# henrycharlesworth/settlers_of_catan_RL

Hardware: AMD Instinct MI355X
Metric: Catan env-steps/sec at 65k parallel games (higher is better)
Workload: dtype u8/u32 (integer bitboards)

## Files before the change

settlers_of_catan_rl_amd/csrc/catan_abi.hip:

```cpp
#include <hip/hip_runtime.h>

#include <cstdio>
#include <cstring>
#include <new>
#include <string>
#include <vector>

#include "../../include/catan_hip.h"
#include "../../include/catan_hip_nn.h"
#include "../../include/catan_hip_tuning.h"
#include "catan_kernels.hip"
#include "catan_obs.hip"
#include "catan_ppo.hip"
#include "catan_nn.hip"
#include "catan_tile_encoder.hip"
#include "catan_heads.hip"
#include "catan_collector.hip"
#include "catan_rows.hip"
#include "catan_te_bwd.hip"
#include "catan_optim.hip"
#include "catan_wgrad_big.hip"

using namespace catan;

struct catan_env {
    int device;
    long n, N;
    Ctx ctx;
    catan_cfg_t cfg;
    void* state;
    u32* mpk;
    u32* spec_state;
    u32* spec_mpk;
    u32 spec_epoch;
    int ctr_clean;
    int lock_parity;
    u32* err;
    double* reward64;
    i32* scratch_actions;
    float* scratch_reward;
    u8* scratch_done;
    Pending pend;
    unsigned long long* prof;
    int prof_on;
    int lr_mid_budget;
    int lr_mid_heavy_grid;
    int t1_group;
    int g_open, g_slot, g_passes; int64_t g_count;
    int lr_split;
    int step_bin_order;
    int step_wpb;
    u32* prof_wave;
    u32* pctr;
    int lr_budget[3];
    int lr_round[2];
    int deferred_fused;
    int fused_subs;
    int step_games;
    hipStream_t side;
    hipEvent_t ev_fork, ev_join;
    hipStream_t fstream[2];
    hipEvent_t ev_fready[3], ev_fdone[3];
    float* f_reward;
    u8* f_done;
    hipStream_t sstream;
    hipEvent_t ev_sdone[2];
    float* s_reward;
    u8* s_done;
    int64_t d_it;
    int d_window;
    hipStream_t d_stream;
    MtPair* mt_dev;
};

constexpr int DEFAULT_STEP_WAVE_GAMES = 32;
constexpr int DEFAULT_FUSED_SUBS = 8;
constexpr int LR_BUDGET_DEFERRED = 12;
constexpr int T1_STAGGER_US = 4, LR_GRID_FUSED = 4096, LR_BUDGET_FUSED = 10;
constexpr unsigned EV_SYNC = hipEventDisableTiming | hipEventDisableSystemFence;
static thread_local std::string g_err;
static int fail(int code, const std::string& msg) { g_err = msg; return code; }
#define HIPCHK(x)                                                                                    \
    do {                                                                                             \
        hipError_t e_ = (x);                                                                         \
        if (e_ != hipSuccess) return fail(CATAN_EHIP, std::string(#x) + ": " + hipGetErrorString(e_)); \
    } while (0)

template <class T>
static int attn_dispatch(bool bwd, const void* qkv, const int* lens, const void* dout, void* out, long B, int L, int H, int HD, hipStream_t st) {
    const T* q = (const T*)qkv;
    const bool mfma = sizeof(T) == 2 && (((uintptr_t)qkv | (uintptr_t)out | (uintptr_t)dout) & 15) == 0;
    const unsigned nb4 = (unsigned)((B + 3) / 4);
    const unsigned short* q16 = (const unsigned short*)qkv;
    if (L == 19 && H == 4 && HD == 16) {
        unsigned nb = (unsigned)((B + 2) / 3);
        if (mfma && !bwd) hipLaunchKernelGGL((k_attn_mfma_fwd<19, 4, 16>), dim3(nb4), dim3(256), 0, st, q16, lens, (unsigned short*)out, B);
        else if (mfma && lens) hipLaunchKernelGGL((k_attn_mfma_bwd<19, 4, 16, true>), dim3(nb4), dim3(256), 0, st, q16, lens, (const unsigned short*)dout, (unsigned short*)out, B);
        else if (mfma) hipLaunchKernelGGL((k_attn_mfma_bwd<19, 4, 16, false>), dim3(nb4), dim3(256), 0, st, q16, lens, (const unsigned short*)dout, (unsigned short*)out, B);
        else if (!bwd) hipLaunchKernelGGL((k_attn_fwd<T, 19, 4, 16>), dim3(nb), dim3(64), 0, st, q, lens, (T*)out, B);
        else hipLaunchKernelGGL((k_attn_bwd<T, 19, 4, 16>), dim3(nb), dim3(64), 0, st, q, lens, (const T*)dout, (T*)out, B);
    } else if (L == 25 && H == 4 && HD == 4) {
        unsigned nb = (unsigned)((B + 1) / 2);
        if (mfma && !bwd) hipLaunchKernelGGL((k_attn_mfma_fwd<25, 4, 4>), dim3(nb4), dim3(256), 0, st, q16, lens, (unsigned short*)out, B);
        else if (mfma && lens) hipLaunchKernelGGL((k_attn_mfma_bwd<25, 4, 4, true>), dim3(nb4), dim3(256), 0, st, q16, lens, (const unsigned short*)dout, (unsigned short*)out, B);
        else if (mfma) hipLaunchKernelGGL((k_attn_mfma_bwd<25, 4, 4, false>), dim3(nb4), dim3(256), 0, st, q16, lens, (const unsigned short*)dout, (unsigned short*)out, B);
        else if (!bwd) hipLaunchKernelGGL((k_attn_fwd<T, 25, 4, 4>), dim3(nb), dim3(64), 0, st, q, lens, (T*)out, B);
        else hipLaunchKernelGGL((k_attn_bwd<T, 25, 4, 4>), dim3(nb), dim3(64), 0, st, q, lens, (const T*)dout, (T*)out, B);
    } else return fail(CATAN_EINVAL, "catan_attention: unsupported (L, heads, head_dim); built for (19,4,16) and (25,4,4)");
    HIPCHK(hipGetLastError());
    return CATAN_OK;
}
template <class T, int D, int GL>
static int ln_launch(bool bwd, const void* x, const float* w, const float* b, const void* dy, void* out, float* dw, float* db,
                     long rows, float eps, int relu, hipStream_t st) {
    long nb = (rows + (256 / GL) - 1) / (256 / GL);
    const long cap = bwd ? 2048 : 8192;
    if (nb > cap) nb = cap;
    if (!bwd) hipLaunchKernelGGL((k_ln_fwd<T, D, GL>), dim3((unsigned)nb), dim3(256), 0, st, (const T*)x, w, b, (T*)out, rows, eps, relu);
    else hipLaunchKernelGGL((k_ln_bwd<T, D, GL>), dim3((unsigned)nb), dim3(256), 0, st, (const T*)x, w, b, (const T*)dy, (T*)out, dw, db, rows, eps, relu);
    HIPCHK(hipGetLastError());
    return CATAN_OK;
}
template <class T, int EPL, int GL>
static int lnw_launch(bool bwd, const void* x, const float* w, const float* b, const void* dy, void* out, float* dw, float* db,
                      long rows, float eps, int relu, hipStream_t st) {
    constexpr int RPB = 256 / GL;
    long nb = (rows + RPB - 1) / RPB;
    const long cap = bwd ? 1024 : 8192;
    if (nb > cap) nb = cap;
// ... 196 lines not shown
    if (cfg) e->cfg = *cfg; else catan_cfg_default(&e->cfg);
    size_t bytes = (size_t)e->N * STATE_BYTES_PER_GAME;
    hipError_t rc = hipMalloc(&e->state, bytes);
    if (rc == hipSuccess) rc = hipMalloc((void**)&e->mpk, (size_t)e->N * MPK_STRIDE * sizeof(u32));
    if (rc == hipSuccess) rc = hipMalloc((void**)&e->spec_state, (size_t)e->N * REC * sizeof(u32));
    if (rc == hipSuccess) rc = hipMalloc((void**)&e->spec_mpk, (size_t)e->N * MPK_STRIDE * sizeof(u32));
    if (rc == hipSuccess) rc = hipMalloc((void**)&e->err, 64);
    if (rc == hipSuccess) rc = hipMalloc((void**)&e->scratch_actions, (size_t)e->n * ACTION_WORDS * sizeof(i32));
    if (rc == hipSuccess) rc = hipMalloc((void**)&e->scratch_reward, (size_t)e->n * 4 * sizeof(float));
    if (rc == hipSuccess) rc = hipMalloc((void**)&e->scratch_done, (size_t)e->n);
    if (rc == hipSuccess) rc = hipMalloc((void**)&e->pend.ctr, CTR_WORDS * sizeof(u32));
    if (rc == hipSuccess) rc = hipMalloc((void**)&e->pend.req[0], (size_t)e->N * sizeof(u64));
    if (rc == hipSuccess) rc = hipMalloc((void**)&e->pend.req[1], (size_t)e->N * sizeof(u64));
    if (rc == hipSuccess) rc = hipMalloc((void**)&e->pend.req[2], (size_t)e->N * sizeof(u64));
    if (rc == hipSuccess) rc = hipMalloc((void**)&e->f_reward, (size_t)e->n * 4 * sizeof(float));
    if (rc == hipSuccess) rc = hipMalloc((void**)&e->f_done, (size_t)e->n);
    int lr_cus = getenv("CATAN_LR_CUS") ? atoi(getenv("CATAN_LR_CUS")) : 0;
    if (rc == hipSuccess && lr_cus > 0) {
        hipDeviceProp_t prop; int dev = 0;
        int cus = (hipGetDevice(&dev) == hipSuccess && hipGetDeviceProperties(&prop, dev) == hipSuccess) ? prop.multiProcessorCount : 256;
        if (lr_cus > cus) lr_cus = cus;
        std::vector<uint32_t> mask((cus + 31) / 32, 0u);
        const char* pat = getenv("CATAN_LR_CUS_PATTERN");
        for (int k = 0; k < lr_cus; k++) { const int b = (pat && pat[0] == 'b') ? k : (int)((long)k * cus / lr_cus); mask[b >> 5] |= 1u << (b & 31); }
        rc = hipExtStreamCreateWithCUMask(&e->fstream[0], (uint32_t)mask.size(), mask.data());
    } else if (rc == hipSuccess) rc = hipStreamCreateWithFlags(&e->fstream[0], hipStreamNonBlocking);
    e->fstream[1] = e->fstream[0];
    for (int i = 0; i < 3 && rc == hipSuccess; i++) {
        rc = hipEventCreateWithFlags(&e->ev_fready[i], EV_SYNC);
        if (rc == hipSuccess) rc = hipEventCreateWithFlags(&e->ev_fdone[i], EV_SYNC);
    }
    for (int i = 0; i < 2 && rc == hipSuccess; i++) {
        rc = hipMalloc((void**)&e->pend.heavy[i], (size_t)e->N * sizeof(u64));
        if (rc == hipSuccess) rc = hipMalloc((void**)&e->pend.resets[i][0], (size_t)e->N * sizeof(i32));
        if (rc == hipSuccess) rc = hipMalloc((void**)&e->pend.resets[i][1], (size_t)e->N * sizeof(i32));
        if (rc == hipSuccess) rc = hipMalloc((void**)&e->pend.resets[i][2], (size_t)e->N * sizeof(i32));
        if (rc == hipSuccess) rc = hipEventCreateWithFlags(&e->ev_sdone[i], EV_SYNC);
    }
    if (rc == hipSuccess) rc = hipMalloc((void**)&e->pend.heavy2, (size_t)e->N * sizeof(u64));
    if (rc == hipSuccess) rc = hipStreamCreateWithFlags(&e->sstream, hipStreamNonBlocking);
    if (rc == hipSuccess) rc = hipMalloc((void**)&e->s_reward, (size_t)e->n * 4 * sizeof(float));
    if (rc == hipSuccess) rc = hipMalloc((void**)&e->s_done, (size_t)e->n);
    e->fused_subs = DEFAULT_FUSED_SUBS;
    if (const char* fs = getenv("CATAN_FUSED_SUBS")) { const int v = atoi(fs); if (v == 1 || v == 2 || v == 4 || v == 8 || v == 16) e->fused_subs = v; }
    static_assert(DEFAULT_FUSED_SUBS <= MAX_SUBS, "sub-lists per bin");
    if (rc == hipSuccess) rc = hipMalloc((void**)&e->pend.lists, (size_t)BIN_SETS * NBINS * e->fused_subs * e->N * sizeof(i32));
    if (rc == hipSuccess) rc = hipMalloc((void**)&e->pend.bctr, (size_t)BIN_SETS * NBINS * MAX_SUBS * BCTR_PAD * sizeof(u32));
    if (rc == hipSuccess) rc = hipStreamCreateWithFlags(&e->side, hipStreamNonBlocking);
    if (rc == hipSuccess) rc = hipEventCreateWithFlags(&e->ev_fork, EV_SYNC);
    if (rc == hipSuccess) rc = hipEventCreateWithFlags(&e->ev_join, EV_SYNC);
    if (rc == hipSuccess) rc = hipMalloc((void**)&e->pend.type, (size_t)e->N);
    if (rc == hipSuccess) rc = hipMalloc((void**)&e->pend.who, (size_t)e->N);
    if (rc == hipSuccess) rc = hipMalloc((void**)&e->pend.len, (size_t)e->N * sizeof(u64));
    if (rc == hipSuccess) rc = hipMalloc((void**)&e->pend.arrive, (size_t)e->N * sizeof(u32));
    if (rc == hipSuccess) rc = hipMalloc((void**)&e->pend.spec, (size_t)e->N * sizeof(u64));
    if (rc == hipSuccess) rc = hipMalloc((void**)&e->pend.busy, (size_t)e->N);
    if (rc == hipSuccess) rc = hipMalloc((void**)&e->pctr, (size_t)e->N * sizeof(u32));
    if (rc == hipSuccess) rc = hipMalloc((void**)&e->prof_wave, (size_t)prof_wave_rows(e->N) * 8 * sizeof(u32));
    if (rc == hipSuccess) rc = hipMalloc((void**)&e->prof, PROF_WORDS * sizeof(unsigned long long));
    if (rc != hipSuccess) { catan_destroy(e); return fail(CATAN_ENOMEM, std::string("catan_create: hipMalloc: ") + hipGetErrorString(rc)); }
    HIPCHK(hipMemset(e->state, 0, bytes));
    HIPCHK(hipMemset(e->err, 0, 64));
    HIPCHK(hipMemset(e->spec_mpk, 0, (size_t)e->N * MPK_STRIDE * sizeof(u32)));
    HIPCHK(hipMemset(e->pend.ctr, 0, CTR_WORDS * sizeof(u32)));
    HIPCHK(hipMemset(e->pend.type, 0, (size_t)e->N));
    HIPCHK(hipMemset(e->pend.busy, 0, (size_t)e->N));
    HIPCHK(hipMemset(e->pend.len, 0, (size_t)e->N * sizeof(u64)));
    HIPCHK(hipMemset(e->pctr, 0, (size_t)e->N * sizeof(u32)));
    e->lr_budget[0] = LR_BUDGET; e->lr_budget[1] = LR_BUDGET_DEFERRED; e->lr_budget[2] = LR_BUDGET_FUSED;
    e->lr_round[0] = LR_ROUND_LOCKSTEP; e->lr_round[1] = LR_ROUND;
    e->step_games = DEFAULT_STEP_WAVE_GAMES;
    e->deferred_fused = 1;
    if (const char* df = getenv("CATAN_DEFERRED_FUSED")) e->deferred_fused = atoi(df) != 0;
    e->step_wpb = 1;
    if (const char* wp = getenv("CATAN_STEP_WAVES_PER_BLOCK")) e->step_wpb = atoi(wp) == 4 ? 4 : 1;
    e->step_bin_order = 1;
    if (const char* bo = getenv("CATAN_STEP_BIN_ORDER")) e->step_bin_order = atoi(bo) != 0;
    e->lr_split = 1;
    e->t1_group = 2;
    if (const char* tg = getenv("CATAN_T1_GROUP")) e->t1_group = atoi(tg) == 1 ? 1 : 2;
    e->lr_mid_budget = 256; e->lr_mid_heavy_grid = 32;
    if (const char* mb = getenv("CATAN_LR_MID_BUDGET")) { e->lr_mid_budget = atoi(mb) > 0 ? atoi(mb) : 0; if (e->lr_mid_budget == 0) e->lr_mid_heavy_grid = 128; }
    if (const char* mg = getenv("CATAN_LR_MID_HEAVY_GRID")) { const int g = atoi(mg); if (g >= 8 && g <= 256) e->lr_mid_heavy_grid = g; }
    if (const char* ls = getenv("CATAN_LR_SPLIT")) e->lr_split = atoi(ls) == 0 ? 0 : (atoi(ls) == 2 ? 2 : 1);
    if (const char* sg = getenv("CATAN_STEP_WAVE_GAMES")) { const int g = atoi(sg); if (g == 64 || g == 32 || g == 16) e->step_games = g; }
    e->pend.fa = 0; e->pend.ftag = 1; e->pend.sa = 0; e->pend.stag = 1; e->pend.sample = 0; e->pend.bnext = 0; e->pend.brel = -1; e->pend.bclear = 1; e->pend.lrq_clear = -1;
    e->pend.nsub = 1;
    HIPCHK(hipMemset(e->pend.bctr, 0, (size_t)BIN_SETS * NBINS * MAX_SUBS * BCTR_PAD * sizeof(u32)));
    HIPCHK(hipMemset(e->mpk, 0, (size_t)e->N * MPK_STRIDE * sizeof(u32)));
    e->ctx.R = (u32*)e->state;
    e->ctx.N = e->N; e->ctx.n = e->n;
    e->ctx.key0 = (u32)seed; e->ctx.key1 = (u32)(seed >> 32);
    e->ctx.env_id0 = env_id0;
    int r = catan_reset(e, nullptr, nullptr);
    if (r != CATAN_OK) { catan_destroy(e); return r; }
    HIPCHK(hipStreamSynchronize(nullptr));
    *out = e;
    return CATAN_OK;
}

void catan_destroy(catan_env_t* e) {
    if (!e) return;
    hipSetDevice(e->device);
    if (e->state) hipFree(e->state);
    if (e->mpk) hipFree(e->mpk);
    if (e->spec_state) hipFree(e->spec_state);
    if (e->spec_mpk) hipFree(e->spec_mpk);
    if (e->err) hipFree(e->err);
    if (e->scratch_actions) hipFree(e->scratch_actions);
    if (e->scratch_reward) hipFree(e->scratch_reward);
    if (e->scratch_done) hipFree(e->scratch_done);
    if (e->prof) hipFree(e->prof);
    if (e->pend.ctr) hipFree(e->pend.ctr);
    if (e->pend.req[0]) hipFree(e->pend.req[0]);
    if (e->pend.req[1]) hipFree(e->pend.req[1]);
    if (e->pend.req[2]) hipFree(e->pend.req[2]);
    if (e->f_reward) hipFree(e->f_reward);
    if (e->f_done) hipFree(e->f_done);
    if (e->fstream[0]) hipStreamDestroy(e->fstream[0]);
    for (int i = 0; i < 3; i++) { if (e->ev_fready[i]) hipEventDestroy(e->ev_fready[i]); if (e->ev_fdone[i]) hipEventDestroy(e->ev_fdone[i]); }
    for (int i = 0; i < 2; i++) {
        if (e->pend.heavy[i]) hipFree(e->pend.heavy[i]);
        if (e->pend.resets[i][0]) hipFree(e->pend.resets[i][0]);
        if (e->pend.resets[i][1]) hipFree(e->pend.resets[i][1]);
        if (e->pend.resets[i][2]) hipFree(e->pend.resets[i][2]);
        if (e->ev_sdone[i]) hipEventDestroy(e->ev_sdone[i]);
    }
    if (e->pend.heavy2) hipFree(e->pend.heavy2);
    if (e->sstream) hipStreamDestroy(e->sstream);
    if (e->s_reward) hipFree(e->s_reward);
    if (e->s_done) hipFree(e->s_done);
    if (e->pend.lists) hipFree(e->pend.lists);
    if (e->pend.bctr) hipFree(e->pend.bctr);
    if (e->mt_dev) hipFree(e->mt_dev);
    if (e->side) hipStreamDestroy(e->side);
    if (e->ev_fork) hipEventDestroy(e->ev_fork);
    if (e->ev_join) hipEventDestroy(e->ev_join);
    if (e->pend.type) hipFree(e->pend.type);
    if (e->pend.who) hipFree(e->pend.who);
    if (e->pend.len) hipFree(e->pend.len);
    if (e->pend.arrive) hipFree(e->pend.arrive);
    if (e->pend.spec) hipFree(e->pend.spec);
    if (e->pend.busy) hipFree(e->pend.busy);
    if (e->pctr) hipFree(e->pctr);
    if (e->prof_wave) hipFree(e->prof_wave);
    delete e;
}

static int deferred_open_error(const catan_env_t* e, const char* what);
#define NOT_DEFERRED(e, what) do { int r_ = deferred_open_error(e, what); if (r_ != CATAN_OK) return r_; } while (0)
static int mt_refill(catan_env_t* e, hipStream_t st) {
    if (e->ctx.mt == nullptr) return CATAN_OK;
    hipLaunchKernelGGL(k_mt_refill, dim3(1), dim3(64), 0, st, e->ctx);
    HIPCHK(hipGetLastError());
    return CATAN_OK;
}
#define NOT_MT(e, what) do { if ((e)->ctx.mt != nullptr) return fail(CATAN_EINVAL, std::string(what) + ": not available for a handle under the MT19937 contract (catan_seed_mt19937)"); } while (0)
int catan_reset(catan_env_t* e, const uint8_t* reset_mask, catan_stream_t stream) {
    if (!e) return fail(CATAN_EINVAL, "catan_reset: null handle");
    NOT_DEFERRED(e, "catan_reset");
    int r = mt_refill(e, S(stream));
    if (r != CATAN_OK) return r;
    hipLaunchKernelGGL(k_reset, dim3((unsigned)(e->N < 16384 ? e->N : 16384)), dim3(64), 0, S(stream), e->ctx, reset_mask, 0);
    HIPCHK(hipGetLastError());
    return launch_masks(e, S(stream));
}
// ... 329 lines not shown
    const bool opens = it % window == 0, last = it + 1 == iters, closes = (it + 1) % window == 0 || last;
    if (it >= D) HIPCHK(hipStreamWaitEvent(st, e->ev_fdone[fa], 0));
    if (it == 0) HIPCHK(hipMemsetAsync(e->pend.ctr, 0, CTR_WORDS * sizeof(u32), st));
    else if (opens) {
        if (w >= 2) HIPCHK(hipStreamWaitEvent(st, e->ev_sdone[sa], 0));
        HIPCHK(hipMemsetAsync(e->pend.ctr + 8 + 4 * sa, 0, 4 * sizeof(u32), st));
    }
    e->pend.fa = fa; e->pend.ftag = ftag; e->pend.sa = sa; e->pend.stag = 4 + sa; e->pend.bsel = ba; e->pend.bclear = ba ^ 1; e->pend.sample = 0; e->pend.brel = -1; e->pend.nsub = 1;
    if (ev) HIPCHK(hipEventRecord(ev[5], st));
    hipLaunchKernelGGL(k_sample_random<BLOCK>, dim3(blocks(e->n, BLOCK)), dim3(BLOCK), 0, st, e->ctx, (const u32*)e->mpk, 0u, e->scratch_actions,
                       e->pctr, e->pend.busy, ftag, (opens && w >= 2) ? 4 + sa : 0, it == 0 ? (u32*)nullptr : e->pend.ctr + (fa < 2 ? 4 + fa : 7), 1,
                       e->pend.ctr + 16 + NBINS * ba, e->pend.lists + (size_t)ba * NBINS * e->N);
    int r = enqueue_fast(e, e->scratch_actions, e->scratch_reward, e->scratch_done, st, ev, true);
    if (r != CATAN_OK) return r;
    static const int extra = getenv("CATAN_DEBUG_EXTRA_EVENTS") ? atoi(getenv("CATAN_DEBUG_EXTRA_EVENTS")) : 0;
    for (int k = 0; k < extra; k++) HIPCHK(hipEventRecord(e->ev_fork, st));
    HIPCHK(hipEventRecord(e->ev_fready[fa], st));
    HIPCHK(hipStreamWaitEvent(e->fstream[0], e->ev_fready[fa], 0));
    r = enqueue_tier1(e, e->f_reward, e->f_done, e->fstream[0], ev, fa, e->lr_budget[1]);
    if (r != CATAN_OK) return r;
    HIPCHK(hipEventRecord(e->ev_fdone[fa], e->fstream[0]));
    if (closes) {
        for (int k = 0; k < D && k <= it; k++) HIPCHK(hipStreamWaitEvent(e->sstream, e->ev_fdone[(fa + D - k) % D], 0));
        r = enqueue_slow(e, e->s_reward, e->s_done, e->sstream, ev, LR_HEAVY_GRID_DEFERRED);
        if (r != CATAN_OK) return r;
        HIPCHK(hipEventRecord(e->ev_sdone[sa], e->sstream));
        if (last) {
            HIPCHK(hipStreamWaitEvent(st, e->ev_sdone[sa], 0));
            if (w >= 1) HIPCHK(hipStreamWaitEvent(st, e->ev_sdone[sa ^ 1], 0));
            hipLaunchKernelGGL(k_release_tags, dim3(blocks(e->N, BLOCK)), dim3(BLOCK), 0, st, e->ctx, e->pend.busy);
            e->pend.fa = 0; e->pend.ftag = 1; e->pend.sa = 0; e->pend.stag = 1;
        }
    }
    return r;
}

static int deferred_iter_grouped(catan_env_t* e, int64_t it, int64_t iters, int window, hipStream_t st, hipEvent_t* ev) {
    constexpr int D = 2;
    const int ba = (int)(it & 1);
    e->ctr_clean = 0;
    const int64_t w = it / window;
    const int sa = (int)(w & 1);
    const bool opens = it % window == 0, last = it + 1 == iters, closes = (it + 1) % window == 0 || last;
    if (it == 0) { e->g_open = 0; e->g_count = 0; }
    const bool g_opens = !e->g_open;
    if (g_opens) { e->g_slot = (int)(e->g_count % D); e->g_passes = 0; e->g_open = 1; }
    const int fa = e->g_slot, ftag = 2 + fa;
    if (g_opens && e->g_count >= D) HIPCHK(hipStreamWaitEvent(st, e->ev_fdone[fa], 0));
    if (it == 0) HIPCHK(hipMemsetAsync(e->pend.ctr, 0, CTR_WORDS * sizeof(u32), st));
    else if (opens) {
        if (w >= 2) HIPCHK(hipStreamWaitEvent(st, e->ev_sdone[sa], 0));
        HIPCHK(hipMemsetAsync(e->pend.ctr + 8 + 4 * sa, 0, 4 * sizeof(u32), st));
    }
    e->pend.fa = fa; e->pend.ftag = ftag; e->pend.sa = sa; e->pend.stag = 4 + sa; e->pend.bsel = ba; e->pend.bclear = ba ^ 1; e->pend.sample = 0; e->pend.brel = -1; e->pend.nsub = 1;
    if (ev) HIPCHK(hipEventRecord(ev[5], st));
    hipLaunchKernelGGL(k_sample_random<512>, dim3(blocks(e->n, 512)), dim3(512), 0, st, e->ctx, (const u32*)e->mpk, 0u, e->scratch_actions,
                       e->pctr, e->pend.busy, g_opens ? ftag : 0, (opens && w >= 2) ? 4 + sa : 0,
                       (g_opens && it != 0) ? e->pend.ctr + 4 + fa : (u32*)nullptr, 1,
                       e->pend.ctr + 16 + NBINS * ba, e->pend.lists + (size_t)ba * NBINS * e->N);
    int r = enqueue_fast(e, e->scratch_actions, e->scratch_reward, e->scratch_done, st, ev, true);
    if (r != CATAN_OK) return r;
    e->g_passes++;
    if (e->g_passes == 2 || closes) {
        HIPCHK(hipEventRecord(e->ev_fready[fa], st));
        HIPCHK(hipStreamWaitEvent(e->fstream[0], e->ev_fready[fa], 0));
        r = enqueue_tier1(e, e->f_reward, e->f_done, e->fstream[0], ev, fa, e->lr_budget[1], true);
        if (r != CATAN_OK) return r;
        HIPCHK(hipEventRecord(e->ev_fdone[fa], e->fstream[0]));
        e->g_open = 0; e->g_count++;
    }
    if (closes) {
        for (int k = 0; k < D && k < e->g_count; k++) HIPCHK(hipStreamWaitEvent(e->sstream, e->ev_fdone[k], 0));
        r = enqueue_slow(e, e->s_reward, e->s_done, e->sstream, ev, LR_HEAVY_GRID_DEFERRED);
        if (r != CATAN_OK) return r;
        HIPCHK(hipEventRecord(e->ev_sdone[sa], e->sstream));
        if (last) {
            HIPCHK(hipStreamWaitEvent(st, e->ev_sdone[sa], 0));
            if (w >= 1) HIPCHK(hipStreamWaitEvent(st, e->ev_sdone[sa ^ 1], 0));
            hipLaunchKernelGGL(k_release_tags, dim3(blocks(e->N, BLOCK)), dim3(BLOCK), 0, st, e->ctx, e->pend.busy);
            e->pend.fa = 0; e->pend.ftag = 1; e->pend.sa = 0; e->pend.stag = 1;
        }
    }
    return r;
}

static int deferred_iter(catan_env_t* e, int64_t it, int64_t iters, int window, hipStream_t st, hipEvent_t* ev) {
    if (!e->deferred_fused && e->t1_group == 2) return deferred_iter_grouped(e, it, iters, window, st, ev);
    if (!e->deferred_fused) return deferred_iter_legacy(e, it, iters, window, st, ev);
    static const int P = (getenv("CATAN_T1_PERIOD") && atoi(getenv("CATAN_T1_PERIOD")) == 1) ? 1 : 2;
    const int S = P + 2;
    const int64_t g = it / P;
    const int ga = (int)(g & 1), gl = (int)(g % 3), rs = (int)(it % S);
    const bool gfirst = it % P == 0, glast = (it + 1) % P == 0;
    e->ctr_clean = 0;
    const int64_t w = it / window;
    const int sa = (int)(w & 1);
    const bool opens = it % window == 0, last = it + 1 == iters, closes = (it + 1) % window == 0 || last;
    if (gfirst && g >= 2) HIPCHK(hipStreamWaitEvent(st, e->ev_fdone[ga], 0));
    if (ev) HIPCHK(hipEventRecord(ev[5], st));
    e->pend.fa = gl; e->pend.ftag = 2 + ga; e->pend.sa = sa; e->pend.stag = 4 + sa;
    e->pend.bsel = rs; e->pend.bnext = (rs + 1) % S; e->pend.bclear = (rs + S - 1) % S; e->pend.sample = 1; e->pend.nsub = e->fused_subs;
    if (it == 0) {
        HIPCHK(hipMemsetAsync(e->pend.ctr, 0, CTR_WORDS * sizeof(u32), st));
        HIPCHK(hipMemsetAsync(e->pend.bctr, 0, (size_t)BIN_SETS * NBINS * MAX_SUBS * BCTR_PAD * sizeof(u32), st));
        hipLaunchKernelGGL(k_sample_first, dim3(blocks(e->N, BLOCK)), dim3(BLOCK), 0, st, e->ctx, e->mpk, (const u32*)e->pctr, e->pend, rs);
    } else if (opens) {
        if (w >= 2) {
            HIPCHK(hipStreamWaitEvent(st, e->ev_sdone[sa], 0));
            hipLaunchKernelGGL(k_release_window, dim3(64), dim3(BLOCK), 0, st, e->ctx, (const u32*)e->mpk, (const u32*)(e->pend.ctr + 11 + 4 * sa),
                               (const i32*)e->pend.resets[sa][2], e->pend, rs);
        }
        HIPCHK(hipMemsetAsync(e->pend.ctr + 8 + 4 * sa, 0, 4 * sizeof(u32), st));
    }
    e->pend.lrq_clear = glast ? (gl + 1) % 3 : -1;
    e->pend.brel = (int)(((g + 2) * P) % S);
    static const int dbg_delay_us = getenv("CATAN_DEBUG_STEP_DELAY_US") ? atoi(getenv("CATAN_DEBUG_STEP_DELAY_US")) : 0;
    if (dbg_delay_us > 0 && closes && !(glast || last)) hipLaunchKernelGGL(k_spin, dim3(1), dim3(64), 0, st, (long long)dbg_delay_us * 100);
    int r = enqueue_fast(e, e->scratch_actions, e->scratch_reward, e->scratch_done, st, ev, true);
    if (r != CATAN_OK) return r;
    if (glast || last) {
        static const bool t1_serial = getenv("CATAN_T1_SERIAL") != nullptr;
        hipStream_t fs = t1_serial ? st : e->fstream[ga];
        HIPCHK(hipEventRecord(e->ev_fready[ga], st));
        HIPCHK(hipStreamWaitEvent(fs, e->ev_fready[ga], 0));
        static const int t1_delay_us = getenv("CATAN_T1_DELAY_US") ? atoi(getenv("CATAN_T1_DELAY_US")) : T1_STAGGER_US;
        const int t1_us = t1_delay_us > 0 && ev != nullptr ? t1_delay_us + 4 : t1_delay_us;
        if (t1_us > 0 && !t1_serial) hipLaunchKernelGGL(k_spin, dim3(1), dim3(64), 0, fs, (long long)t1_us * 100);
        r = enqueue_tier1(e, e->f_reward, e->f_done, fs, ev, gl, e->lr_budget[2], false, LR_GRID_FUSED);
        if (r != CATAN_OK) return r;
        HIPCHK(hipEventRecord(e->ev_fdone[ga], fs));
    }
    if (closes) {
        HIPCHK(hipStreamWaitEvent(e->sstream, e->ev_fdone[ga], 0));
        if (g >= 1) HIPCHK(hipStreamWaitEvent(e->sstream, e->ev_fdone[ga ^ 1], 0));
        static const bool dbg_unordered = getenv("CATAN_DEBUG_FUSED_CLOSE_UNORDERED") != nullptr;
        if (!(glast || last) && !dbg_unordered) {
            HIPCHK(hipEventRecord(e->ev_fready[2], st));
            HIPCHK(hipStreamWaitEvent(e->sstream, e->ev_fready[2], 0));
        }
        e->pend.brel = -1;
        r = enqueue_slow(e, e->s_reward, e->s_done, e->sstream, ev, LR_HEAVY_GRID_DEFERRED);
        if (r != CATAN_OK) return r;
        HIPCHK(hipEventRecord(e->ev_sdone[sa], e->sstream));
        if (last) {
            HIPCHK(hipStreamWaitEvent(st, e->ev_sdone[sa], 0));
            if (w >= 1) HIPCHK(hipStreamWaitEvent(st, e->ev_sdone[sa ^ 1], 0));
            hipLaunchKernelGGL(k_finish_rollout, dim3(blocks(e->N, BLOCK)), dim3(BLOCK), 0, st, e->ctx, (const u32*)e->mpk, e->pctr, e->pend.busy);
            e->pend.fa = 0; e->pend.ftag = 1; e->pend.sa = 0; e->pend.stag = 1; e->pend.sample = 0; e->pend.nsub = 1;
        }
    }
    return r;
}

int catan_random_rollout_deferred(catan_env_t* e, int64_t iters, int32_t window, catan_stream_t stream) {
    if (!e || iters < 0 || window <= 0) return fail(CATAN_EINVAL, "catan_random_rollout_deferred: bad arguments");
    NOT_DEFERRED(e, "catan_random_rollout_deferred");
    NOT_MT(e, "catan_random_rollout_deferred");
    for (int64_t it = 0; it < iters; it++) {
        int r = deferred_iter(e, it, iters, window, S(stream), nullptr);
        if (r != CATAN_OK) return r;
    }
    return CATAN_OK;
}

static int deferred_open_error(const catan_env_t* e, const char* what) {
    if (e && e->d_it > 0) return fail(CATAN_EINVAL, std::string(what) + ": a deferred step sequence is open (call catan_step_flush first)");
    return CATAN_OK;
}
int catan_step_deferred(catan_env_t* e, const int32_t* actions, int32_t window, float* reward, uint8_t* done, uint8_t* status, catan_stream_t stream) {
    if (!e || !actions || !reward || !done || !status || window <= 0) return fail(CATAN_EINVAL, "catan_step_deferred: bad arguments");
    NOT_MT(e, "catan_step_deferred");
    hipStream_t st = S(stream);
    if (e->d_it > 0 && (window != e->d_window || st != e->d_stream))
        return fail(CATAN_EINVAL, "catan_step_deferred: window and stream must stay the same between two flushes");
    const int64_t it = e->d_it;
    const int fa = (int)(it & 1);
    const int64_t w = it / window;
    const int sa = (int)(w & 1);
    const bool opens = it % window == 0, closes = (it + 1) % window == 0;
    e->ctr_clean = 0;
    e->d_window = window; e->d_stream = st;
    if (it == 0) HIPCHK(hipMemsetAsync(e->pend.ctr, 0, CTR_WORDS * sizeof(u32), st));
    else if (opens) HIPCHK(hipMemsetAsync(e->pend.ctr + 8 + 4 * sa, 0, 4 * sizeof(u32), st));
    e->pend.fa = fa; e->pend.ftag = 2 + fa; e->pend.sa = sa; e->pend.stag = 4 + sa; e->pend.bsel = fa; e->pend.bclear = fa ^ 1; e->pend.sample = 0; e->pend.brel = -1; e->pend.nsub = 1;
    hipLaunchKernelGGL(k_classify_deferred, dim3(blocks(e->N, BLOCK)), dim3(BLOCK), 0, st, e->ctx, actions, (const u8*)e->pend.busy, e->pend.ctr + 16 + NBINS * fa,
                       e->pend.lists + (size_t)fa * NBINS * e->N, it == 0 ? (u32*)nullptr : e->pend.ctr + 4 + fa, 1, e->cfg.validate_actions ? e->err : (u32*)nullptr);
    int r = enqueue_fast(e, actions, e->f_reward, e->f_done, st, nullptr, true);
    if (r != CATAN_OK) return r;
    HIPCHK(hipEventRecord(e->ev_fready[fa], st));
    HIPCHK(hipStreamWaitEvent(e->fstream[fa], e->ev_fready[fa], 0));
    r = enqueue_tier1(e, e->f_reward, e->f_done, e->fstream[fa], nullptr, fa, e->lr_budget[1]);
    if (r != CATAN_OK) return r;
    HIPCHK(hipEventRecord(e->ev_fdone[fa], e->fstream[fa]));
    if (closes) {
        HIPCHK(hipStreamWaitEvent(e->sstream, e->ev_fdone[fa], 0));
        if (it >= 1) HIPCHK(hipStreamWaitEvent(e->sstream, e->ev_fdone[fa ^ 1], 0));
        r = enqueue_slow(e, e->f_reward, e->f_done, e->sstream, nullptr, LR_HEAVY_GRID_DEFERRED);
        if (r != CATAN_OK) return r;
        HIPCHK(hipEventRecord(e->ev_sdone[sa], e->sstream));
    }
    const int64_t nit = it + 1, nw = nit / window;
    const bool nopens = nit % window == 0;
    if (nit >= 2) HIPCHK(hipStreamWaitEvent(st, e->ev_fdone[nit & 1], 0));
    if (nopens && nw >= 2) HIPCHK(hipStreamWaitEvent(st, e->ev_sdone[nw & 1], 0));
    hipLaunchKernelGGL(k_deliver, dim3(blocks(e->n, BLOCK)), dim3(BLOCK), 0, st, e->ctx, e->pend.busy, nit >= 2 ? 2 + (int)(nit & 1) : 0, (nopens && nw >= 2) ? 4 + (int)(nw & 1) : 0, 0,
                       (const float*)e->f_reward, (const u8*)e->f_done, reward, done, status);
    HIPCHK(hipGetLastError());
    e->d_it = nit;
    return CATAN_OK;
}

int catan_step_flush(catan_env_t* e, float* reward, uint8_t* done, uint8_t* status, catan_stream_t stream) {
    if (!e || !reward || !done || !status) return fail(CATAN_EINVAL, "catan_step_flush: null argument");
// ... 839 lines not shown
```

settlers_of_catan_rl_amd/csrc/catan_kernels.hip:

```cpp
#include <hip/hip_runtime.h>
#include <stdint.h>

#include "catan_state.h"

#define CATAN_TABLE static __device__ __constant__ const
#define CATAN_FN static __device__ __forceinline__
#define CATAN_TOPOLOGY_CODE
#include "catan_topology.inc"

namespace catan {

#define DEVI __device__ __forceinline__

constexpr int BLOCK = 256;
constexpr u64 ALL54 = (1ull << 54) - 1;

constexpr int MT_RING = 8192, MT_AHEAD = 6144, MT_AHEAD_PY = 1024;
struct MtGen { u32 mt[624]; u32 idx; u32 produced; u32 ring[MT_RING]; };
struct MtPair { MtGen np, py; u32 cons_py; };
struct Ctx {
    u32* R;
    long N;
    long n;
    u32 key0, key1;
// ... 2433 lines not shown
        for (int i = 0; i < 4; i++) dst[i] = make_uint4((u32)a[4 * i], (u32)a[4 * i + 1], (u32)a[4 * i + 2], (u32)a[4 * i + 3]);
        dst[4] = make_uint4((u32)a[16], (u32)a[17], d, 0u);
    }
    u32 rank = 0;
    const bool valid = s.e < c.n;
    if (valid) rank = atomicAdd(&hist[bin], 1u);
    __syncthreads();
    const int sub = (int)(blockIdx.x & (pend.nsub - 1));
    if (threadIdx.x < NBINS) base[threadIdx.x] = hist[threadIdx.x] ? atomicAdd(sub_ctr(pend, set, threadIdx.x, sub), hist[threadIdx.x]) : 0u;
    __syncthreads();
    if (valid) sub_list(pend, set, bin, sub, c.N)[base[bin] + rank] = (i32)s.e;
}
__global__ __launch_bounds__(BLOCK) void k_release_window(Ctx c, const u32* __restrict__ mpk, const u32* __restrict__ count_p, const i32* __restrict__ list,
                                                         Pending pend, int set) {
    const u32 count = *count_p;
    for (u32 r = blockIdx.x * BLOCK + threadIdx.x; r < count; r += gridDim.x * BLOCK) {
        const long e = list[r];
        const u32* row = mpk + e * MPK_STRIDE;
        const int bin = bin_of((int)row[ROW_ACT], (int)row[ROW_ACT + 4]), sub = (int)(e & (pend.nsub - 1));
        sub_list(pend, set, bin, sub, c.N)[atomicAdd(sub_ctr(pend, set, bin, sub), 1u)] = (i32)e;
    }
}
__global__ __launch_bounds__(BLOCK) void k_finish_rollout(Ctx c, const u32* __restrict__ mpk, u32* __restrict__ pctr, u8* __restrict__ busy) {
    const long e = (long)blockIdx.x * BLOCK + threadIdx.x;
    if (e < c.n) pctr[e] = mpk[e * MPK_STRIDE + ROW_CTR];
    if (e < c.N) busy[e] = 0;
}

DEVI void wave_reset_game(const Ctx& c, long e, u32* rec, ResetScratch& sc, int lane, u32* __restrict__ mpk, Limits lim, u8* busy,
                           unsigned long long* prof = nullptr, u32* __restrict__ dstR = nullptr, const Pending* pend = nullptr, bool board_only = false) {
    u32* const outR = dstR ? dstR : c.R;
    __builtin_amdgcn_wave_barrier();
    if (lane < ROWS_HOT / 4) reinterpret_cast<uint4*>(rec)[lane] = reinterpret_cast<const uint4*>(c.R + e * REC)[lane];
    __builtin_amdgcn_wave_barrier();
    StL1 s(rec, outR, c.N, e);
    Rng mine = rng_load(c, s);
    const u32 blk0 = mine.draws >> 2;
#pragma unroll
    for (int b = 0; b < RND_WORDS / 256; b++) {
        u32 o[4];
        mine.block(blk0 + b * 64 + lane, o);
        const int at = (b * 64 + lane) * 4;
        sc.rnd[at] = o[0]; sc.rnd[at + 1] = o[1]; sc.rnd[at + 2] = o[2]; sc.rnd[at + 3] = o[3];
    }
    for (int r = ROWS_HOT + lane; r < REC; r += 64) outR[e * REC + r] = 0;
    __builtin_amdgcn_wave_barrier();
    RngBuf rb;
    rb.buf = sc.rnd; rb.base = blk0 * 4; rb.avail = RND_WORDS; rb.slow = mine;
    const long long t0 = prof ? wall_clock64() : 0;
    if (lane == 0) reset_part1(s, rb, sc, ROWS_HOT);
    __builtin_amdgcn_wave_barrier();
    const bool tokens_done = reset_tokens_parallel(sc, lane);
    __builtin_amdgcn_wave_barrier();
    if (lane == 0) {
        reset_part2(s, rb, sc, tokens_done, board_only);
        if (prof) {
            const unsigned long long dt = (unsigned long long)(wall_clock64() - t0);
            atomicAdd(&prof[5], dt); atomicMax(&prof[PROF_PHASES + 5], dt);
            atomicAdd(&prof[3], (unsigned long long)(rb.slow.draws - mine.draws)); atomicMax(&prof[PROF_PHASES + 3], (unsigned long long)(rb.slow.draws - mine.draws));
            atomicAdd(&prof[4], 1ull);
        }
        if (mpk != nullptr) {
            u32 m[MASK_WORDS];
            compute_masks(s, m, lim);
#pragma unroll
            for (int i = 0; i < MASK_WORDS; i++) mpk[e * MPK_STRIDE + i] = m[i];
            if (pend != nullptr && pend->sample) sample_enqueue_lane(c, s, m, *pend, mpk);
        }
    }
    __builtin_amdgcn_wave_barrier();
    if (lane < ROWS_HOT / 4) reinterpret_cast<uint4*>(outR + e * REC)[lane] = reinterpret_cast<const uint4*>(rec)[lane];
    if (lane == 0 && busy != nullptr) busy[e] = 0;
}
__global__ __launch_bounds__(64) void k_reset_list(Ctx c, u32* __restrict__ mpk, Limits lim, const u32* __restrict__ count_p,
                                                   const i32* __restrict__ list, u8* __restrict__ busy, unsigned long long* prof,
                                                   const u32* __restrict__ spec_count_p, const u64* __restrict__ spec_list,
                                                   u32* __restrict__ specR, u32* __restrict__ spec_mpk, u32 epoch, Pending pend) {
    __shared__ __attribute__((aligned(16))) u32 rec[ROWS_HOT];
    __shared__ ResetScratch sc;
    const u32 count = *count_p, scount = spec_list ? *spec_count_p : 0u;
    for (u32 r = blockIdx.x; r < count + scount; r += gridDim.x) {
        if (r < count) wave_reset_game(c, list[r], rec, sc, threadIdx.x, mpk, lim, busy, prof, nullptr, &pend);
        else {
            const long e = (long)(spec_list[r - count] & 0x00FFFFFFFFFFFFFFull);
            wave_reset_game(c, e, rec, sc, threadIdx.x, spec_mpk, lim, nullptr, nullptr, specR);
            if (threadIdx.x == 0) spec_mpk[e * MPK_STRIDE + MPK_STRIDE - 1] = epoch;
        }
    }
}
__global__ __launch_bounds__(64) void k_install_list(Ctx c, u32* __restrict__ mpk, Limits lim, const u32* __restrict__ count_p,
                                                     const i32* __restrict__ list, u8* __restrict__ busy, const u32* __restrict__ specR,
                                                     const u32* __restrict__ spec_mpk, u32 epoch, u32* __restrict__ err) {
    __shared__ __attribute__((aligned(16))) u32 rec[ROWS_HOT];
    __shared__ ResetScratch sc;
    const u32 count = *count_p;
    const int lane = threadIdx.x;
    for (u32 r = blockIdx.x; r < count; r += gridDim.x) {
        const long e = list[r];
        if (spec_mpk[e * MPK_STRIDE + MPK_STRIDE - 1] != epoch) {
            if (lane == 0) atomicAdd(err + 2, 1u);
            wave_reset_game(c, e, rec, sc, lane, mpk, lim, busy, nullptr);
            continue;
        }
        if (lane < REC / 4) reinterpret_cast<uint4*>(c.R + e * REC)[lane] = reinterpret_cast<const uint4*>(specR + e * REC)[lane];
        if (lane < 3)
            reinterpret_cast<uint4*>(mpk + e * MPK_STRIDE)[lane] = reinterpret_cast<const uint4*>(spec_mpk + e * MPK_STRIDE)[lane];
        if (lane == 0 && busy != nullptr) busy[e] = 0;
    }
}
__global__ __launch_bounds__(64) void k_reset(Ctx c, const u8* __restrict__ sel, int board_only) {
    __shared__ __attribute__((aligned(16))) u32 rec[ROWS_HOT];
    __shared__ ResetScratch sc;
    for (long e = blockIdx.x; e < c.N; e += gridDim.x) {
        if (sel != nullptr && (e >= c.n || sel[e] == 0)) continue;
        wave_reset_game(c, e, rec, sc, threadIdx.x, nullptr, Limits{ -1, -1 }, nullptr, nullptr, nullptr, nullptr, board_only != 0);
    }
}
__global__ __launch_bounds__(64) void k_mt_refill(Ctx c) {
    if (threadIdx.x != 0 || c.mt == nullptr) return;
    MtPair& m = *c.mt;
    const u32 want_np = c.R[W_RNG] + (u32)MT_AHEAD, want_py = m.cons_py + (u32)MT_AHEAD_PY;
    while ((int)(want_np - m.np.produced) > 0) { m.np.ring[m.np.produced & (u32)(MT_RING - 1)] = mt_next(m.np); m.np.produced++; }
    while ((int)(want_py - m.py.produced) > 0) { m.py.ring[m.py.produced & (u32)(MT_RING - 1)] = mt_next(m.py); m.py.produced++; }
}

DEVI int action_bin(const Ctx& c, const i32* __restrict__ actions, long e) {
    if (e >= c.n) return BIN_NOOP;
    return bin_of(actions[e * ACTION_WORDS], actions[e * ACTION_WORDS + 4]);
}
DEVI void sort_append(long e, bool valid, int bin, u32* hist, u32* base, u32* __restrict__ bins, i32* __restrict__ lists, long N) {
    u32 rank = 0;
    if (valid) rank = atomicAdd(&hist[bin], 1u);
    __syncthreads();
    if (threadIdx.x < NBINS) base[threadIdx.x] = hist[threadIdx.x] ? atomicAdd(&bins[threadIdx.x], hist[threadIdx.x]) : 0u;
    __syncthreads();
    if (valid) lists[(long)bin * N + base[bin] + rank] = (i32)e;
}
__global__ __launch_bounds__(BLOCK) void k_classify(Ctx c, const i32* __restrict__ actions, u32* __restrict__ bins, i32* __restrict__ lists,
                                                    u32* __restrict__ zero_me, int zero_n, u32* __restrict__ err) {
    __shared__ u32 hist[NBINS], base[NBINS];
    if (threadIdx.x < NBINS) hist[threadIdx.x] = 0;
    __syncthreads();
    const long e = (long)blockIdx.x * BLOCK + threadIdx.x;
    if (zero_me != nullptr && e < zero_n) zero_me[e] = 0;
    if (err != nullptr && e < c.n && actions[e * ACTION_WORDS] > 12) atomicAdd(err, 1u);
    sort_append(e, e < c.n, e < c.n ? action_bin(c, actions, e) : BIN_NOOP, hist, base, bins, lists, c.N);
}
__global__ __launch_bounds__(BLOCK) void k_classify_deferred(Ctx c, const i32* __restrict__ actions, const u8* __restrict__ busy, u32* __restrict__ bins,
                                                             i32* __restrict__ lists, u32* __restrict__ zero_me, int zero_n, u32* __restrict__ err) {
    __shared__ u32 hist[NBINS], base[NBINS];
    if (threadIdx.x < NBINS) hist[threadIdx.x] = 0;
    __syncthreads();
    const long e = (long)blockIdx.x * BLOCK + threadIdx.x;
    if (zero_me != nullptr && e < zero_n) zero_me[e] = 0;
    const bool plays = e < c.n && busy[e] == 0;
    if (err != nullptr && plays && actions[e * ACTION_WORDS] > 12) atomicAdd(err, 1u);
    sort_append(e, plays, plays ? action_bin(c, actions, e) : BIN_NOOP, hist, base, bins, lists, c.N);
}
__global__ __launch_bounds__(BLOCK) void k_deliver(Ctx c, u8* __restrict__ busy, int tag_a, int tag_b, int release_all, const float* __restrict__ res_reward,
                                                   const u8* __restrict__ res_done, float* __restrict__ reward, u8* __restrict__ done, u8* __restrict__ status) {
    const long e = (long)blockIdx.x * BLOCK + threadIdx.x;
    if (e >= c.n) return;
    int b = busy[e];
    const bool was_waiting = b != 0;
    if (b != 0 && (release_all || (b >= 2 && (b == tag_a || b == tag_b)))) { busy[e] = 0; b = 0; }
    const bool deliver = b == 0 && (!release_all || was_waiting);
    float4 r = make_float4(0.f, 0.f, 0.f, 0.f);
// ... 353 lines not shown
```

Baseline: 1.059 billion.

## Close final rollout window on tier-1 stream instead of separate slow-stream drain

On the last iteration of a deferred fused rollout, the final slow-path close (reset list, LR finish/heavy, install list) now runs directly on the tier-1 stream right after tier-1 work, rather than handing off to the separate slow stream and its event waits. This removes a cross-stream handoff and serialization at the rollout tail. The old path is kept behind an environment flag. It risks subtle ordering bugs around event dependencies and the reused heavy2 counter, and a constant mask is replaced with a named one.

```diff
diff --git a/settlers_of_catan_rl_amd/csrc/catan_abi.hip b/settlers_of_catan_rl_amd/csrc/catan_abi.hip
--- a/settlers_of_catan_rl_amd/csrc/catan_abi.hip
+++ b/settlers_of_catan_rl_amd/csrc/catan_abi.hip
@@ -45,6 +45,7 @@
     int prof_on;
     int lr_mid_budget;
     int lr_mid_heavy_grid;
+    int drain_legacy;
     int t1_group;
     int g_open, g_slot, g_passes; int64_t g_count;
     int lr_split;
@@ -407,6 +408,8 @@
     e->lr_mid_budget = 256; e->lr_mid_heavy_grid = 32;
     if (const char* mb = getenv("CATAN_LR_MID_BUDGET")) { e->lr_mid_budget = atoi(mb) > 0 ? atoi(mb) : 0; if (e->lr_mid_budget == 0) e->lr_mid_heavy_grid = 128; }
     if (const char* mg = getenv("CATAN_LR_MID_HEAVY_GRID")) { const int g = atoi(mg); if (g >= 8 && g <= 256) e->lr_mid_heavy_grid = g; }
+    e->drain_legacy = 0;
+    if (const char* dl = getenv("CATAN_DRAIN_LEGACY")) e->drain_legacy = atoi(dl) != 0;
     if (const char* ls = getenv("CATAN_LR_SPLIT")) e->lr_split = atoi(ls) == 0 ? 0 : (atoi(ls) == 2 ? 2 : 1);
     if (const char* sg = getenv("CATAN_STEP_WAVE_GAMES")) { const int g = atoi(sg); if (g == 64 || g == 32 || g == 16) e->step_games = g; }
     e->pend.fa = 0; e->pend.ftag = 1; e->pend.sa = 0; e->pend.stag = 1; e->pend.sample = 0; e->pend.bnext = 0; e->pend.brel = -1; e->pend.bclear = 1; e->pend.lrq_clear = -1;
@@ -902,6 +905,39 @@
         }
     }
     return r;
+}
+
+static int final_close(catan_env_t* e, hipStream_t fs, hipEvent_t* ev) {
+    StepCfg sc = step_cfg(e);
+    const int sa = e->pend.sa; const Limits lim = limits_of(e);
+    u32* sctr = e->pend.ctr + 8 + 4 * sa;
+    if (e->cfg.auto_reset) {
+        e->spec_epoch++;
+        HIPCHK(hipEventRecord(e->ev_fork, fs));
+        HIPCHK(hipStreamWaitEvent(e->side, e->ev_fork, 0));
+        hipLaunchKernelGGL(k_reset_list, dim3(RESET_GRID), dim3(64), 0, e->side, e->ctx, e->mpk, lim, (const u32*)(sctr + 1), (const i32*)e->pend.resets[sa][0],
+                           (u8*)nullptr, sc.prof, (const u32*)sctr, (const u64*)e->pend.heavy[sa], e->spec_state, e->spec_mpk, e->spec_epoch, e->pend);
+        HIPCHK(hipEventRecord(e->ev_join, e->side));
+    }
+    if (ev) HIPCHK(hipEventRecord(ev[9], fs));
+    if (e->lr_mid_budget > 0) {
+        hipLaunchKernelGGL(k_lr_finish<LRF_MID>, dim3(LR_MID_GRID), dim3(64), 0, fs, e->ctx, e->mpk, e->s_reward, e->s_done, sc, e->pend, 0, e->lr_mid_budget,
+                           (unsigned long long*)nullptr, (unsigned long long*)nullptr);
+        hipLaunchKernelGGL(k_lr_heavy, dim3(LR_HEAVY_GRID), dim3(LR_HEAVY_THREADS), 0, fs, e->ctx, (const u32*)(e->pend.ctr + CTR_HEAVY2), (const u64*)e->pend.heavy2,
+                           e->pend.len, e->lr_round[0], e->mpk, e->s_reward, e->s_done, sc, e->pend);
+    } else
+        hipLaunchKernelGGL(k_lr_heavy, dim3(LR_HEAVY_GRID), dim3(LR_HEAVY_THREADS), 0, fs, e->ctx, (const u32*)sctr, (const u64*)e->pend.heavy[sa],
+                           e->pend.len, e->lr_round[0], e->mpk, e->s_reward, e->s_done, sc, e->pend);
+    if (ev) HIPCHK(hipEventRecord(ev[3], fs));
+    if (ev) HIPCHK(hipEventRecord(ev[7], fs));
+    if (e->cfg.auto_reset) {
+        HIPCHK(hipStreamWaitEvent(fs, e->ev_join, 0));
+        hipLaunchKernelGGL(k_install_list, dim3(256), dim3(64), 0, fs, e->ctx, e->mpk, lim, (const u32*)(sctr + 2), (const i32*)e->pend.resets[sa][1], (u8*)nullptr,
+                           (const u32*)e->spec_state, (const u32*)e->spec_mpk, e->spec_epoch, e->err);
+    }
+    if (ev) HIPCHK(hipEventRecord(ev[4], fs));
+    HIPCHK(hipGetLastError());
+    return CATAN_OK;
 }
 
 static int deferred_iter(catan_env_t* e, int64_t it, int64_t iters, int window, hipStream_t st, hipEvent_t* ev) {
@@ -945,10 +981,27 @@
         HIPCHK(hipStreamWaitEvent(fs, e->ev_fready[ga], 0));
         static const int t1_delay_us = getenv("CATAN_T1_DELAY_US") ? atoi(getenv("CATAN_T1_DELAY_US")) : T1_STAGGER_US;
         const int t1_us = t1_delay_us > 0 && ev != nullptr ? t1_delay_us + 4 : t1_delay_us;
+        const bool fast_close = last && !e->drain_legacy;
+        if (fast_close) {
+            if (w >= 1) HIPCHK(hipStreamWaitEvent(fs, e->ev_sdone[sa ^ 1], 0));
+            if (g >= 1 && fs != st) HIPCHK(hipStreamWaitEvent(fs, e->ev_fdone[ga ^ 1], 0));
+            HIPCHK(hipMemsetAsync(e->pend.ctr + CTR_HEAVY2, 0, sizeof(u32), fs));
+        }
         if (t1_us > 0 && !t1_serial) hipLaunchKernelGGL(k_spin, dim3(1), dim3(64), 0, fs, (long long)t1_us * 100);
         r = enqueue_tier1(e, e->f_reward, e->f_done, fs, ev, gl, e->lr_budget[2], false, LR_GRID_FUSED);
         if (r != CATAN_OK) return r;
         HIPCHK(hipEventRecord(e->ev_fdone[ga], fs));
+        if (fast_close) {
+            e->pend.brel = -1;
+            r = final_close(e, fs, ev);
+            if (r != CATAN_OK) return r;
+            HIPCHK(hipEventRecord(e->ev_sdone[sa], fs));
+            HIPCHK(hipStreamWaitEvent(st, e->ev_sdone[sa], 0));
+            hipLaunchKernelGGL(k_finish_rollout, dim3(blocks(e->N, BLOCK)), dim3(BLOCK), 0, st, e->ctx, (const u32*)e->mpk, e->pctr, e->pend.busy);
+            e->pend.fa = 0; e->pend.ftag = 1; e->pend.sa = 0; e->pend.stag = 1; e->pend.sample = 0; e->pend.nsub = 1;
+            HIPCHK(hipGetLastError());
+            return CATAN_OK;
+        }
     }
     if (closes) {
         HIPCHK(hipStreamWaitEvent(e->sstream, e->ev_fdone[ga], 0));
diff --git a/settlers_of_catan_rl_amd/csrc/catan_kernels.hip b/settlers_of_catan_rl_amd/csrc/catan_kernels.hip
--- a/settlers_of_catan_rl_amd/csrc/catan_kernels.hip
+++ b/settlers_of_catan_rl_amd/csrc/catan_kernels.hip
@@ -2539,7 +2539,7 @@
     for (u32 r = blockIdx.x; r < count + scount; r += gridDim.x) {
         if (r < count) wave_reset_game(c, list[r], rec, sc, threadIdx.x, mpk, lim, busy, prof, nullptr, &pend);
         else {
-            const long e = (long)(spec_list[r - count] & 0x00FFFFFFFFFFFFFFull);
+            const long e = (long)(spec_list[r - count] & LR_GAME_MASK);
             wave_reset_game(c, e, rec, sc, threadIdx.x, spec_mpk, lim, nullptr, nullptr, specR);
             if (threadIdx.x == 0) spec_mpk[e * MPK_STRIDE + MPK_STRIDE - 1] = epoch;
         }
```

New measurement: 1.060 billion, median of 6. No clear change (+0.1%).
